# speechcatcher-asr/speechcatcher

Measured on AMD Instinct MI355X. Metric: concurrent real-time streams (audio-seconds/s), de_xl dims, 640 ms (10240-sample) chunk steps, beam 10 CTC+attention, higher is better.
Workload: dtype f32

## Files before the change

include/scasr.h:

```cpp
#ifndef SCASR_H
#define SCASR_H

#include <stddef.h>
#include <stdint.h>

#ifdef __cplusplus
extern "C" {
#endif

#define SC_OK 0
#define SC_ERR_ARG (-1)
#define SC_ERR_LAUNCH (-2)
#define SC_ERR_CAPACITY (-3)
#define SC_ERR_INPUT (-4)

#define SC_GEMM_RELU 1
#define SC_GEMM_RESIDUAL 2
#define SC_GEMM_LN_AT_CROWS 8
#define SC_GEMM_NAIVE 4
#define SC_GEMM_SPLIT16 16

#define SC_F_ANY_EOS 1
#define SC_F_BEST_EOS 2
#define SC_F_ALL_EOS 4
// ... 321 lines not shown
int sc_align_hyps(sc_streams *streams, const int *stream_ids, int n, int nbest, int max_len, int32_t *start,
                  int32_t *end, float *logp_mean, double *path_score, int *status, int *n_hyps);
int sc_align_tokens(sc_streams *streams, int stream, const int32_t *ids, int L, int32_t *start, int32_t *end,
                    float *logp_mean, double *path_score, int *status);
int sc_reset(sc_streams *streams, int stream);
int sc_stream_info(const sc_streams *streams, int stream, sc_stream_info_t *out);
#define SC_KV_POOL_DEFAULT_MAX_GIB 24
int sc_streams_kv_rows(const sc_streams *streams);
int sc_streams_stats(const sc_streams *streams, long *enc_calls, long *dec_steps, long *dec_blocks);
int sc_streams_capture_stats(const sc_streams *streams, long *n_captures, double *seconds);
int sc_streams_set_graphs(sc_streams *streams, int on);
int sc_marker(int id, void *stream);
int sc_streams_host_times(sc_streams *streams, double *launch_s, double *wait_s);
int sc_streams_bucket_times(sc_streams *streams, double *seconds, long *iterations);
long sc_streams_take_xattn_rows(sc_streams *streams);
int sc_streams_take_xattn_rows_by_kernel(sc_streams *streams, long *rows);
int sc_streams_take_attn_counters(sc_streams *streams, long *out );
void *sc_streams_hip_stream(sc_streams *streams);
float *sc_streams_pcm(sc_streams *streams, long *capacity);
int sc_streams_write_pcm(sc_streams *streams, int stream, long offset, const float *host, long n);
long sc_streams_read_pcm_buffer(sc_streams *streams, int stream, float *host, long max_n);
int sc_streams_read_enc(sc_streams *streams, int stream, float *host, int max_frames);
int sc_streams_read_ctc(sc_streams *streams, int stream, float *host, int max_rows);

#ifdef __cplusplus
}
#endif
#endif
```

speechcatcher_amd/_abi.py:

```python
import ctypes as C
import os
import subprocess
from pathlib import Path

HERE = Path(__file__).resolve().parent
LIB_PATH = HERE / "libscasr.so"
CSRC = HERE / "csrc"

c_float_p = C.POINTER(C.c_float)
c_int_p = C.POINTER(C.c_int32)
c_double_p = C.POINTER(C.c_double)
vp = C.c_void_p


class EncLayer(C.Structure):
    _fields_ = [(n, vp) for n in ("ln1_g", "ln1_b", "wqkv", "bqkv", "wo", "bo",
                                  "ln2_g", "ln2_b", "w1", "b1", "w2", "b2", "w1_p", "w2_p",
                                  "wqkv_p", "wo_p", "w1_h", "w2_h", "wqkv_h", "wo_h", "w1_s", "w2_s",
                                  "wqkv_s", "wo_s")]


class DecLayer(C.Structure):
    _fields_ = [(n, vp) for n in ("ln1_g", "ln1_b", "wqkv", "bqkv", "wo", "bo",
                                  "ln2_g", "ln2_b", "wq", "bq", "wo2", "bo2",
# ... 154 lines not shown
    "sc_stream_last_error": (C.c_char_p, [vp, C.c_int]),
    "sc_reset": (C.c_int, [vp, C.c_int]),
    "sc_stream_info": (C.c_int, [vp, C.c_int, C.POINTER(StreamInfo)]),
    "sc_streams_stats": (C.c_int, [vp, C.POINTER(C.c_long), C.POINTER(C.c_long), C.POINTER(C.c_long)]),
    "sc_streams_capture_stats": (C.c_int, [vp, C.POINTER(C.c_long), c_double_p]),
    "sc_streams_set_graphs": (C.c_int, [vp, C.c_int]),
    "sc_marker": (C.c_int, [C.c_int, vp]),
    "sc_streams_host_times": (C.c_int, [vp, c_double_p, c_double_p]),
    "sc_streams_bucket_times": (C.c_int, [vp, c_double_p, C.POINTER(C.c_long)]),
    "sc_streams_take_xattn_rows": (C.c_long, [vp]),
    "sc_streams_take_xattn_rows_by_kernel": (C.c_int, [vp, vp]),
    "sc_streams_take_attn_counters": (C.c_int, [vp, vp]),
    "sc_streams_hip_stream": (vp, [vp]),
    "sc_streams_pcm": (vp, [vp, C.POINTER(C.c_long)]),
    "sc_streams_write_pcm": (C.c_int, [vp, C.c_int, C.c_long, vp, C.c_long]),
    "sc_streams_read_pcm_buffer": (C.c_long, [vp, C.c_int, vp, C.c_long]),
    "sc_streams_read_enc": (C.c_int, [vp, C.c_int, vp, C.c_int]),
    "sc_ctc_align_ws_bytes": (C.c_size_t, [C.c_int]),
    "sc_ctc_align": (C.c_int, [vp, C.c_int, C.c_int, C.c_int, vp]),
    "sc_align_hyps": (C.c_int, [vp, c_int_p, C.c_int, C.c_int, C.c_int, c_int_p, c_int_p, c_float_p, c_double_p,
                                c_int_p, c_int_p]),
    "sc_align_tokens": (C.c_int, [vp, C.c_int, c_int_p, C.c_int, c_int_p, c_int_p, c_float_p, c_double_p, c_int_p]),
    "sc_streams_read_ctc": (C.c_int, [vp, C.c_int, vp, C.c_int]),
}

EXPORTED_SYMBOLS = tuple(_SIGS.keys())

ABI_VERSION = 7

_lib = None


class ScasrError(RuntimeError):
    pass


def build(verbose: bool = False) -> Path:
    cmd = ["make", "-C", str(CSRC), "-j4"]
    res = subprocess.run(cmd, capture_output=True, text=True)
    if verbose or res.returncode != 0:
        print(res.stdout)
        print(res.stderr)
    if res.returncode != 0:
        raise ScasrError("building libscasr.so failed")
    return LIB_PATH

# ... 32 lines not shown
```

speechcatcher_amd/csrc/common.h:

```cpp
#pragma once
#include <hip/hip_runtime.h>
#include <stdint.h>
#include <stdio.h>
#include <math.h>

#include "../../include/scasr.h"

#define SC_LOGZERO (-10000000000.0f)

void sc_set_error(const char *fmt, ...);

const char *sc_hook(const char *name);

__attribute__((visibility("hidden"))) int allow_large_lds(const void *fn, size_t need, size_t max_bytes, const char *what);

#define SC_CHECK_ARG(cond, msg)      \
  do {                               \
    if (!(cond)) {                   \
      sc_set_error("%s: %s", __func__, msg); \
      return SC_ERR_ARG;             \
    }                                \
  } while (0)

#define SC_CHECK_LAUNCH()                                              \
// ... 16 lines not shown
  __attribute__((visibility("hidden"))) ~ProfScope() {
    if (on) { (void)hipEventDestroy(a); (void)hipEventDestroy(b); }
  }
};
ProfScope sc_prof_begin(hipStream_t st);
void sc_prof_end(ProfScope &p, int kind, double flops, double bytes);

int sc_decode_step_form(const sc_search *sb);
int sc_gemm_colblocks(const float *A, const int32_t *a_rows, int lda, const float *W, const float *bias, float *C,
                      const int32_t *c_rows, int ldc, int M, int N, int K, int ncb, long cb_stride, int flags, void *stream);

int sc_dec_layer_hpw(const sc_search &sb);
int sc_dec_layer_stream_form(const sc_search &sb);
int sc_dec_layer_split_ffn(const sc_search &sb);

int sc_launch_reduce_ln_proj(const float *part, int npart, int part_M, const float *b2, const float *Xin, float *Xout,
                             const int32_t *rows, int M, int D, const float *ln_g, const float *ln_b, float ln_eps,
                             float *XN, const float *Wq, const float *bq, float *Q, int N, hipStream_t st,
                             int by_row = 0, int half_mode = 0);

struct ScHandoff { const int32_t *blkinfo; int R; float *state; int layer; };
int sc_ffn_ln_handoff(const float *XN, int M, int D, int F, const void *W1, const float *b1, const void *W2, const float *b2,
                      float *X, int w_form, const ScHandoff &ho, void *stream);

template <int CTRL>
__device__ __forceinline__ float dpp_mov(float v) {
  return __int_as_float(__builtin_amdgcn_update_dpp(0, __float_as_int(v), CTRL, 0xF, 0xF, true));
}
#define SC_DPP_XOR1 0xB1
#define SC_DPP_XOR2 0x4E
#define SC_DPP_HALF_MIRROR 0x141
#define SC_DPP_ROR4 0x124
#define SC_DPP_ROR8 0x128
#define SC_DPP_ROW_MIRROR 0x140

template <int LPR>
__device__ __forceinline__ float group_sum(float v) {
  v += dpp_mov<SC_DPP_XOR1>(v);
  v += dpp_mov<SC_DPP_XOR2>(v);
  if (LPR >= 8) v += dpp_mov<SC_DPP_HALF_MIRROR>(v);
  if (LPR == 16) v += dpp_mov<SC_DPP_ROW_MIRROR>(v);
  return v;
}

__device__ __forceinline__ float sc_lane(float v, int lane) {
  return __int_as_float(__builtin_amdgcn_readlane(__float_as_int(v), lane));
// ... 108 lines not shown
```

speechcatcher_amd/csrc/encoder.hip:

```cpp
#include "common.h"
#include <stdarg.h>
#include <string.h>

static thread_local char g_err[512] = "";
void sc_set_error(const char *fmt, ...) {
  va_list ap;
  va_start(ap, fmt);
  vsnprintf(g_err, sizeof(g_err), fmt, ap);
  va_end(ap);
}
extern "C" const char *sc_last_error(void) { return g_err; }
extern "C" int sc_version(void) { return SC_ABI_VERSION; }

template <int ID>
__global__ void sc_marker_kernel() {}
extern "C" int sc_marker(int id, void *stream) {
  hipStream_t st = (hipStream_t)stream;
  switch (id) {
    case 0: sc_marker_kernel<0><<<1, 64, 0, st>>>(); break;
    case 1: sc_marker_kernel<1><<<1, 64, 0, st>>>(); break;
    case 2: sc_marker_kernel<2><<<1, 64, 0, st>>>(); break;
    case 3: sc_marker_kernel<3><<<1, 64, 0, st>>>(); break;
    default: sc_set_error("sc_marker: id must be 0..3"); return SC_ERR_ARG;
  }
// ... 563 lines not shown
  const bool mfma = dk == 32 && R <= 48 && !(masked && R < 2) && !sp;
  if (mfma) {
    enc_attention_mfma_kernel<<<nblk * H, 256, 0, st>>>(qkv, att, nblk, R, H, d, masked);
  } else if (dk == 32 && split) {
    enc_attention_split_kernel<32><<<nblk * H, 256, 4 * 64 * (32 + 2) * sizeof(float), st>>>(qkv, att, nblk, R, H, d,
                                                                                            masked);
  } else if (dk == 16 && split) {
    enc_attention_split_kernel<16><<<nblk * H, 256, 4 * 64 * (16 + 2) * sizeof(float), st>>>(qkv, att, nblk, R, H, d,
                                                                                            masked);
  } else if (dk == 32) {
    enc_attention_kernel<32><<<grid, 256, 4 * 2 * 64 * 32 * sizeof(float), st>>>(qkv, att, nblk, R, H, d, masked);
  } else if (dk == 16) {
    enc_attention_kernel<16><<<grid, 256, 4 * 2 * 64 * 16 * sizeof(float), st>>>(qkv, att, nblk, R, H, d, masked);
  } else if (dk == 64) {
    enc_attention_kernel<64><<<grid, 256, 4 * 2 * 64 * 64 * sizeof(float), st>>>(qkv, att, nblk, R, H, d, masked);
  } else {
    sc_set_error("sc_enc_attention: unsupported head dim %d", dk);
    return SC_ERR_ARG;
  }
  SC_CHECK_LAUNCH();
  return SC_OK;
}

extern "C" int sc_encoder_layers(const sc_enc_layer *L, int n_layers, float *x, int nblk, int R,
                                 int masked, const int32_t *jobs, int ns, float *past_ctx,
                                 float *xn, float *qkv, float *att, float *ffh, int d, int H, int F,
                                 float eps, void *stream) {
  SC_CHECK_ARG(L && x && xn && qkv && att && ffh, "null pointer");
  const int M = nblk * R;
  if (M <= 0) return SC_OK;
  const bool ffn_fused = sc_ffn_ln_supported(d, F) && sc_workspace_bytes(stream) >= (size_t)(F / 128) * 80 * d * sizeof(float);
  const char *re = sc_hook("SC_ENC_ROWTILE");
  const bool rowtile_ok = sc_rowtile_proj_supported(d, d) && !(re && atoi(re) == 0);
  int rc;
  const bool fused_handoff = masked && ns > 0 && ffn_fused && R > 1 &&
                             sc_workspace_bytes(stream) >= (size_t)(F / 128) * M * d * sizeof(float) &&
                             (size_t)M * F >= (size_t)nblk * 4;
  int32_t *blkinfo = reinterpret_cast<int32_t *>(ffh);
  if (fused_handoff) {
    ctx_blkinfo_kernel<<<1, 256, 0, (hipStream_t)stream>>>(jobs, ns, nblk, blkinfo);
    SC_CHECK_LAUNCH();
  }
  for (int li = 0; li < n_layers; ++li) {
    const sc_enc_layer &w = L[li];
    const bool rowtile = rowtile_ok && w.wqkv_p && w.wo_p;
    const bool proj_h = rowtile && w.wqkv_h && w.wo_h;
    const bool proj_s = rowtile && w.wqkv_s && w.wo_s;
    if (proj_s) {
      SC_TRY(sc_rowtile_proj_s(x, d, M, d, w.ln1_g, w.ln1_b, eps, w.wqkv_s, w.bqkv, 3 * d, nullptr, qkv, 3 * d,
                               nullptr, nullptr, nullptr, stream));
    } else if (proj_h) {
      SC_TRY(sc_rowtile_proj_h(x, d, M, d, w.ln1_g, w.ln1_b, eps, w.wqkv_h, w.bqkv, 3 * d, nullptr, qkv, 3 * d,
                               nullptr, nullptr, nullptr, stream));
    } else if (rowtile) {
      SC_TRY(sc_rowtile_proj(x, d, M, d, w.ln1_g, w.ln1_b, eps, w.wqkv_p, w.bqkv, 3 * d, nullptr, qkv, 3 * d,
                             nullptr, nullptr, nullptr, stream));
    } else {
      SC_TRY(sc_layernorm(x, nullptr, d, xn, nullptr, d, M, d, w.ln1_g, w.ln1_b, eps, stream));
      SC_TRY(sc_gemm(xn, nullptr, d, w.wqkv, w.bqkv, qkv, nullptr, 3 * d, M, 3 * d, d, 0, 0, stream));
    }
    SC_TRY(sc_enc_attention(qkv, att, nblk, R, H, d, masked, stream));
    if (proj_s) {
      SC_TRY(sc_rowtile_proj_s(att, d, M, d, nullptr, nullptr, eps, w.wo_s, w.bo, d, x, x, d, w.ln2_g, w.ln2_b, xn,
                               stream));
    } else if (proj_h) {
      SC_TRY(sc_rowtile_proj_h(att, d, M, d, nullptr, nullptr, eps, w.wo_h, w.bo, d, x, x, d, w.ln2_g, w.ln2_b, xn,
                               stream));
    } else if (rowtile) {
      SC_TRY(sc_rowtile_proj(att, d, M, d, nullptr, nullptr, eps, w.wo_p, w.bo, d, x, x, d, w.ln2_g, w.ln2_b, xn,
                             stream));
    } else {
      SC_TRY(sc_gemm(att, nullptr, d, w.wo, w.bo, x, nullptr, d, M, d, d, SC_GEMM_RESIDUAL, 0, stream));
      SC_TRY(sc_layernorm(x, nullptr, d, xn, nullptr, d, M, d, w.ln2_g, w.ln2_b, eps, stream));
    }
    if (fused_handoff) {
      const int wf = (w.w1_s && w.w2_s) ? 2 : (w.w1_h && w.w2_h) ? 1 : 0;
      const ScHandoff ho{blkinfo, R, past_ctx, li};
      SC_TRY(sc_ffn_ln_handoff(xn, M, d, F, wf == 2 ? w.w1_s : wf == 1 ? w.w1_h : (const void *)w.w1_p, w.b1,
                               wf == 2 ? w.w2_s : wf == 1 ? w.w2_h : (const void *)w.w2_p, w.b2, x, wf, ho, stream));
      continue;
    }
    if (ffn_fused) {
      if (w.w1_s && w.w2_s)
        SC_TRY(sc_ffn_ln_s(xn, nullptr, M, d, F, w.w1_s, w.b1, w.w2_s, w.b2, x, nullptr, nullptr, eps, nullptr, stream));
      else if (w.w1_h && w.w2_h)
        SC_TRY(sc_ffn_ln_h(xn, nullptr, M, d, F, w.w1_h, w.b1, w.w2_h, w.b2, x, nullptr, nullptr, eps, nullptr, stream));
      else
        SC_TRY(sc_ffn_ln(xn, nullptr, M, d, F, w.w1_p, w.b1, w.w2_p, w.b2, x, nullptr, nullptr, eps, nullptr, stream));
    } else {
      SC_TRY(sc_gemm(xn, nullptr, d, w.w1, w.b1, ffh, nullptr, F, M, F, d, SC_GEMM_RELU, 0, stream));
      SC_TRY(sc_gemm(ffh, nullptr, F, w.w2, w.b2, x, nullptr, d, M, d, F, SC_GEMM_RESIDUAL, 0, stream));
    }
    if (masked && ns > 0) SC_TRY(sc_ctx_handoff(x, R, jobs, ns, past_ctx, li, d, stream));
  }
  return SC_OK;
}
```

speechcatcher_amd/csrc/streams.hip:

```cpp
#include <algorithm>
#include <array>
#include <chrono>
#include <cmath>
#include <cstdarg>
#include <cstring>
#include <deque>
#include <map>
#include <memory>
#include <new>
#include <string>
#include <vector>

#include "common.h"

namespace {

#define HIP_TRY(call)                                                              \
  do {                                                                             \
    hipError_t e__ = (call);                                                       \
    if (e__ != hipSuccess) {                                                       \
      sc_set_error("%s: %s failed: %s", __func__, #call, hipGetErrorString(e__));  \
      return SC_ERR_LAUNCH;                                                        \
    }                                                                              \
  } while (0)
// ... 119 lines not shown
  size_t stage_floats = 0;
  std::vector<int32_t> fe_jobs;
  int n_fe = 0, max_keep = 0;
  EncPlan P;
  std::vector<int32_t> ctc_rows, kv_src, kv_dst;
  bool same_rows = true;
  std::vector<int> streams;
  bool empty() const { return !n_fe && !P.n_conv; }
};

constexpr int N_ARENA = 8;
constexpr int N_STAGE = 4;
constexpr int N_RING = 4;

struct sc_streams {
  sc_engine *eng = nullptr;
  sc_config cfg{};
  int S = 0, W = 0, K = 0, TCAP = 0, LCAP = 0, FCAP = 0, UCAP = 0, max_feat_new = 0, max_t1 = 0, max_t2 = 0,
      max_blocks = 0, max_chunk = 0, max_length = 500;
  long PCAP = 0;
  bool use_bbd = false, strict = true;
  hipStream_t stream = nullptr;
  hipStream_t stream_enc = nullptr, es = nullptr;
  hipEvent_t ev_iter[2] = {nullptr, nullptr};
  int32_t *ring_dev = nullptr;
  int32_t *rm_host[2] = {nullptr, nullptr};
  int rm_idx = 0;
  bool rm_dirty = false;
  int scan_split_min = 1024, scan_split_streams = 0;
  bool scan_long = false;
  int step_split_min() const { return (scan_long && (scan_split_streams <= 0 || n_rows_step <= scan_split_streams * W)) ? scan_split_min : 0; }
  int graph_key() const { return n_rows_step * 2 + (step_split_min() > 0 ? 1 : 0); }
  int enc_start_thr = 0;
  int enc_batch_min = 0;
  int gemm_flags = 0;
  void *ws = nullptr, *ws_enc = nullptr;
  std::vector<void *> owned, owned_host;
  float *pcm = nullptr, *featbuf = nullptr, *subbuf = nullptr, *prev_addin = nullptr, *past_ctx = nullptr, *enc = nullptr,
        *c1 = nullptr, *c2 = nullptr, *xblk = nullptr, *ws_xn = nullptr, *ws_qkv = nullptr, *ws_att = nullptr,
        *ws_ffh = nullptr;
  int32_t *jobs_ctx = nullptr, *ctrlmap = nullptr;
  float *kv_stage = nullptr;
  int kv_stage_rows = 0;
  sc_search sb{};
  int32_t *ctrlmap_host = nullptr, *flags_host = nullptr;
  int32_t *arena_host = nullptr, *arena_dev = nullptr;
  size_t slot_cap = 0, arena_off = 0;
  int cur_slot = 0;
  hipEvent_t ev_group[N_ARENA] = {nullptr};
  long slot_gen[N_ARENA] = {0};
  int32_t *bs_host = nullptr, *bs_dev = nullptr;
  size_t bs_cap = 0;
  int bs_i = 0;
  float *stage_host = nullptr, *stage_dev = nullptr;
  size_t stage_cap = 0;
  hipEvent_t ev_stage[N_STAGE] = {nullptr};
  bool stage_busy[N_STAGE] = {false};
  int stage_next = 0;
  long long *cjobs_host = nullptr, *cjobs_dev = nullptr;
// ... 28 lines not shown
  std::vector<int> rowmap_key;
  int row_bucket = 1, n_rows_step = 0;
  bool decode_prepared = false;
  std::map<int, hipGraphExec_t> dec_graphs;
  std::map<std::vector<long>, hipGraphExec_t> enc_graphs;
  long dec_steps = 0, dec_blocks = 0, enc_calls = 0, xattn_rows[3] = {0, 0, 0};
  long sattn_pos[3] = {0, 0, 0};
  unsigned long long *stat_rows = nullptr;
  double t_launch = 0, t_wait = 0;
  double t_bucket[17] = {0};
  long n_bucket[17] = {0};
  bool use_graphs = true;
  long n_enc_captures = 0;
  double t_enc_capture = 0;

  ~sc_streams() {
    for (auto &g : dec_graphs) (void)hipGraphExecDestroy(g.second);
    for (auto &g : enc_graphs) (void)hipGraphExecDestroy(g.second);
    if (stream) (void)sc_set_stream_workspace(stream, nullptr, 0);
    if (stream_enc) {
      (void)sc_set_stream_workspace(stream_enc, nullptr, 0);
      (void)hipStreamDestroy(stream_enc);
    }
    for (int i = 0; i < 2; ++i)
      if (ev_iter[i]) (void)hipEventDestroy(ev_iter[i]);
    for (int i = 0; i < N_ARENA; ++i)
      if (ev_group[i]) (void)hipEventDestroy(ev_group[i]);
    for (int i = 0; i < N_STAGE; ++i)
      if (ev_stage[i]) (void)hipEventDestroy(ev_stage[i]);
    if (ev_snap) (void)hipEventDestroy(ev_snap);
    for (EncGroup *g : groups) delete g;
    for (void *p : owned) (void)hipFree(p);
    for (void *p : owned_host) (void)hipHostFree(p);
    if (stream_rb) (void)hipStreamDestroy(stream_rb);
    if (stream) (void)hipStreamDestroy(stream);
    if (al_dev) (void)hipFree(al_dev);
  }

  template <typename T>
  int alloc(T **p, size_t n) {
    RC_TRY(dalloc(p, n));
    owned.push_back(*p);
    return SC_OK;
  }
  template <typename T>
  int halloc(T **p, size_t n) {
// ... 267 lines not shown
    for (int i = 0; i < nb; ++i) {
      const int cur_hop = i * c.hop_size + (first ? offset : 0);
      const int clen = (i == nb - 1 && fin) ? std::min(c.block_size - offset, y_len - cur_hop) : c.hop_size;
      for (int j = 0; j < clen; ++j)
        if (cur_hop + j >= 0 && cur_hop + j < y_len) src[cur_hop + j] = (b0 + i) * R + 1 + offset + j;
    }
    if (st.T_enc + y_len > b->TCAP) throw StreamFault{s, SC_ERR_CAPACITY, "encoder-frame capacity exceeded (max_frames)"};
    for (int i = 0; i < y_len; ++i) {
      P.emit_src.push_back(src[i]);
      P.emit_dst.push_back(s * b->TCAP + st.T_enc + i);
    }
    st.T_enc += y_len;
    st.n_blocks += nb;
  }
  for (int s : streams)
    if (finals.at(s)) {
      St &st = b->st[s];
      st.enc_started = false;
      st.nfeat = st.nsub = st.n_blocks = 0;
      st.has_sub = st.has_addin = st.has_ctx = false;
    }
}

int enc_layers_launch(sc_streams *b, int nblk, int R, bool masked, const int32_t *jobs, int ns) {
  const sc_config &c = b->cfg;
  sc_engine *e = b->eng;
  auto launch = [&]() {
    return sc_encoder_layers(e->enc.data(), (int)e->enc.size(), b->xblk, nblk, R, masked ? 1 : 0, jobs, ns, b->past_ctx,
                             b->ws_xn, b->ws_qkv, b->ws_att, b->ws_ffh, c.d_model, c.enc_heads, c.ffn_dim, c.ln_eps,
                             b->es);
  };
  if (!b->use_graphs) return launch();
  std::vector<long> key{nblk, R, (long)masked, (long)(intptr_t)jobs, ns};
  auto it = b->enc_graphs.find(key);
  if (it == b->enc_graphs.end()) {
    if (b->enc_graphs.size() >= 192) return launch();
    const auto tc0 = std::chrono::steady_clock::now();
    RC_TRY(sc_graph_capture_begin(b->es));
    const int rc = launch();
    void *g = nullptr;
    const int rc2 = sc_graph_capture_end(b->es, &g);
    b->n_enc_captures++;
    b->t_enc_capture += std::chrono::duration<double>(std::chrono::steady_clock::now() - tc0).count();
    if (rc != SC_OK) return rc;
    if (rc2 != SC_OK) return rc2;
    it = b->enc_graphs.emplace(key, (hipGraphExec_t)g).first;
  }
  return sc_graph_launch(it->second, b->es);
}

int encode_short(sc_streams *b, const EncPlan::Short &sh) {
  const sc_config &c = b->cfg;
  sc_engine *e = b->eng;
  const int U = sh.U;
  const int32_t *jd, *src, *dst;
  RC_TRY(b->itensor({sh.ubase, U, sh.pe_pos, 0, 1, 0}, &jd));
  RC_TRY(sc_block_pack(b->subbuf, jd, 1, U, e->f("pe"), c.d_model, b->xblk, b->es));
  RC_TRY(sc_encoder_layers(e->enc.data(), (int)e->enc.size(), b->xblk, 1, U, 0, nullptr, 0, b->past_ctx, b->ws_xn,
                           b->ws_qkv, b->ws_att, b->ws_ffh, c.d_model, c.enc_heads, c.ffn_dim, c.ln_eps, b->es));
  std::vector<int32_t> a(U), d(U);
  for (int i = 0; i < U; ++i) { a[i] = i; d[i] = sh.s * b->TCAP + sh.dst_T + i; }
  RC_TRY(b->itensor(a, &src));
  RC_TRY(b->itensor(d, &dst));
  RC_TRY(sc_layernorm(b->xblk, src, c.d_model, b->enc, dst, c.d_model, U, c.d_model, e->f("enc_norm_g"), e->f("enc_norm_b"),
                      c.ln_eps, b->es));
  return SC_OK;
}

int encode_launch(sc_streams *b, EncPlan &P) {
  const sc_config &c = b->cfg;
  sc_engine *e = b->eng;
// ... 11 lines not shown
  if (!P.feat_src.empty()) {
    const int32_t *a, *z;
    RC_TRY(b->itensor(P.feat_src, &a));
    RC_TRY(b->itensor(P.feat_dst, &z));
    RC_TRY(sc_copy_rows(b->featbuf, a, b->featbuf, z, (int)P.feat_src.size(), c.n_mels, b->es));
  }
  const int nbk = (int)P.blk_jobs.size() / 6, ns = (int)P.sjobs.size() / 5;
  if (nbk > 0) {
    if (nbk > b->max_blocks) {
      sc_set_error("sc_push: too many encoder blocks in one call");
      return SC_ERR_ARG;
    }
    const int32_t *bj, *ja;
    RC_TRY(b->itensor(P.blk_jobs, &bj));
    RC_TRY(sc_block_pack(b->subbuf, bj, nbk, R, e->f("pe"), d, b->xblk, b->es));
    std::vector<int32_t> j_add(ns * 4), j_ctx(ns * 4);
    for (int i = 0; i < ns; ++i) {
      const int32_t *sj = &P.sjobs[i * 5];
      j_add[i * 4 + 0] = sj[0]; j_add[i * 4 + 1] = sj[1]; j_add[i * 4 + 2] = sj[2]; j_add[i * 4 + 3] = sj[3];
      j_ctx[i * 4 + 0] = sj[0]; j_ctx[i * 4 + 1] = sj[1]; j_ctx[i * 4 + 2] = sj[2] * c.enc_layers; j_ctx[i * 4 + 3] = sj[4];
    }
    RC_TRY(b->itensor(j_add, &ja));
    RC_TRY(sc_ctx_handoff(b->xblk, R, ja, ns, b->prev_addin, 0, d, b->es));
    const int32_t *jc;
    RC_TRY(b->itensor(j_ctx, &jc));
    HIP_TRY(hipMemcpyAsync(b->jobs_ctx, jc, j_ctx.size() * sizeof(int32_t), hipMemcpyDeviceToDevice, b->es));
    RC_TRY(enc_layers_launch(b, nbk, R, true, b->jobs_ctx, ns));
  }
  if (!P.emit_src.empty()) {
    const int32_t *a, *z;
    RC_TRY(b->itensor(P.emit_src, &a));
    RC_TRY(b->itensor(P.emit_dst, &z));
    RC_TRY(sc_layernorm(b->xblk, a, d, b->enc, z, d, (int)P.emit_src.size(), d, e->f("enc_norm_g"), e->f("enc_norm_b"),
                        c.ln_eps, b->es));
  }
  for (auto &sh : P.shorts) RC_TRY(encode_short(b, sh));
  if (!P.sub_src.empty()) {
    const int32_t *a, *z;
    RC_TRY(b->itensor(P.sub_src, &a));
    RC_TRY(b->itensor(P.sub_dst, &z));
    RC_TRY(sc_copy_rows(b->subbuf, a, b->subbuf, z, (int)P.sub_src.size(), d, b->es));
  }
  return SC_OK;
}

void set_rowmap(sc_streams *b, const std::vector<int> &active) {
  const int S = b->S, W = b->W;
  const int na = (int)active.size();
  const int nb = std::min(S, (na + b->row_bucket - 1) / b->row_bucket * b->row_bucket);
  if (active != b->rowmap_key) {
// ... 903 lines not shown
  if (hipStreamCreateWithPriority(&b->stream, hipStreamNonBlocking, -1) != hipSuccess) {
    sc_set_error("sc_streams_create: hipStreamCreate failed");
    delete b;
    return SC_ERR_LAUNCH;
  }
  if (hipStreamCreateWithPriority(&b->stream_rb, hipStreamNonBlocking, -1) != hipSuccess) {
    sc_set_error("sc_streams_create: hipStreamCreate failed");
    delete b;
    return SC_ERR_LAUNCH;
  }
  A(b->pcm, (size_t)S * b->PCAP);
  A(b->featbuf, (size_t)2 * S * b->FCAP * c.n_mels);
  A(b->subbuf, (size_t)2 * S * b->UCAP * d);
  A(b->prev_addin, (size_t)S * d);
  A(b->past_ctx, (size_t)S * c.enc_layers * d);
  A(b->enc, (size_t)S * b->TCAP * d);
  A(b->c1, (size_t)S * b->max_t1 * c.conv_freq1 * d);
  A(b->c2, (size_t)S * b->max_t2 * c.conv_freq2 * d);
  A(b->xblk, m_enc * d);
  A(b->ws_xn, m_enc * d);
  A(b->ws_qkv, m_enc * 3 * d);
  A(b->ws_att, m_enc * d);
  A(b->ws_ffh, m_enc * F);
  A(b->jobs_ctx, (size_t)S * 4);
  A(b->ctrlmap, (size_t)S * 8 + n);
  b->slot_cap = (((size_t)S * ((size_t)b->max_t2 * (c.conv_freq2 + 12) + 512) + 8192) + 63) & ~size_t(63);
  A(b->arena_dev, b->slot_cap * N_ARENA);
  b->bs_cap = (size_t)S * 8 + (size_t)S * c.block_size;
  A(b->bs_dev, b->bs_cap * N_RING);
  b->stage_cap = (size_t)S * std::max<size_t>((size_t)b->max_chunk + 16 * c.hop_length, (size_t)b->max_feat_new * c.n_mels);
  A(b->stage_dev, b->stage_cap * N_STAGE);
  b->pack_cap = n * (2 * (size_t)b->LCAP + 8);
  A(b->pack_dev, b->pack_cap);
  A(b->pjobs_dev, n * 4);
  A(b->cjobs_dev, (size_t)N_STAGE * S * 3);
  sc_search &sb = b->sb;
  sb.S = S; sb.W = W; sb.K = K; sb.V = V; sb.d = d; sb.H = c.dec_heads; sb.F = F; sb.n_layers = c.dec_layers;
  sb.TCAP = b->TCAP; sb.LCAP = b->LCAP; sb.blank = c.blank_id; sb.eos = c.eos_id; sb.sos = c.sos_id;
  sb.w_dec = 1.0f - o->ctc_weight; sb.w_ctc = o->ctc_weight; sb.ln_eps = c.ln_eps;
  float *ctcx = nullptr, *ckv = nullptr;
  A(ctcx, (size_t)S * b->TCAP * V);
  sb.kv_half = o->kv_half != 0;
  const size_t kvdiv = sb.kv_half ? 2 : 1;
  A(ckv, (size_t)S * c.dec_layers * b->TCAP * 2 * d / kvdiv + 4);
  sb.ctcx = ctcx; sb.ckv = ckv;
  if (sb.kv_half) {
    b->kv_stage_rows = std::max(256, S * 24);
// ... 67 lines not shown
  if (sb.kv_half && e->f("out_w_qh", false) && !e->dec.empty() && e->dec[0].wqkv_pph && e->dec[0].wq_pph && e->dec[0].wo_pph &&
      e->dec[0].wo2_pph && sb.ph1) {
    sb.out_w_qh = e->f("out_w_qh", false);
    sb.act_half = 1 | 2;
    if (const char *ah = sc_hook("SC_ACT_HALF")) sb.act_half = atoi(ah) & 7;
  }
  sb.layers = e->dec.data();
  (void)sc_set_stream_workspace(b->stream, b->ws, (size_t)128 << 20);
  b->es = b->stream;
  {
    b->enc_start_thr = S < 16 ? S : std::max(1, (int)((long)S * 7 / 100));
  }
  {
    const hipError_t er = hipStreamCreateWithPriority(&b->stream_enc, hipStreamNonBlocking, 0);
    if (er == hipSuccess && hipMalloc(&b->ws_enc, (size_t)128 << 20) == hipSuccess) {
      b->owned.push_back(b->ws_enc);
      (void)sc_set_stream_workspace(b->stream_enc, b->ws_enc, (size_t)128 << 20);
    } else {
      (void)hipGetLastError();
      if (b->stream_enc) (void)hipStreamDestroy(b->stream_enc);
      b->stream_enc = nullptr;
    }
  }
  const size_t cm = ((size_t)S * 8 + n) * sizeof(int32_t);
  bool ok = b->halloc(&b->ctrlmap_host, (size_t)S * 8 + n) == SC_OK && b->halloc(&b->flags_host, (size_t)S * 2) == SC_OK &&
            b->halloc(&b->rm_host[0], n) == SC_OK && b->halloc(&b->rm_host[1], n) == SC_OK &&
            b->halloc(&b->arena_host, b->slot_cap * N_ARENA) == SC_OK && b->halloc(&b->bs_host, b->bs_cap * N_RING) == SC_OK &&
            b->halloc(&b->stage_host, b->stage_cap * N_STAGE) == SC_OK && b->halloc(&b->pack_host, b->pack_cap) == SC_OK &&
            b->halloc(&b->pjobs_host, n * 4) == SC_OK && b->halloc(&b->cjobs_host, (size_t)N_STAGE * S * 3) == SC_OK;
  for (int i = 0; i < 2 && ok; ++i) ok = hipEventCreateWithFlags(&b->ev_iter[i], hipEventDisableTiming) == hipSuccess;
  for (int i = 0; i < N_ARENA && ok; ++i) ok = hipEventCreateWithFlags(&b->ev_group[i], hipEventDisableTiming) == hipSuccess;
  for (int i = 0; i < N_STAGE && ok; ++i) ok = hipEventCreateWithFlags(&b->ev_stage[i], hipEventDisableTiming) == hipSuccess;
  if (!ok) {
    sc_set_error("sc_streams_create: pinned host allocation failed");
    delete b;
    return SC_ERR_LAUNCH;
  }
  memset(b->flags_host, 0, (size_t)S * 8);
  {
    void *dv = nullptr;
    if (hipHostGetDevicePointer(&dv, b->flags_host, 0) != hipSuccess || !dv) {
      sc_set_error("sc_streams_create: pinned flags are not device-accessible");
      delete b;
      return SC_ERR_LAUNCH;
    }
    b->ring_dev = (int32_t *)dv;
// ... 11 lines not shown
  b->gemm_flags = (!b->eng->enc.empty() && b->eng->enc[0].wqkv_s) ? SC_GEMM_SPLIT16 : 0;
  b->row_bucket = std::max(1, S / 32);
  b->n_rows_step = S * W;
  b->st.assign(S, St());
  b->run.assign(S, Run());
  b->bq.assign(S, std::deque<Blk>());
  b->job.assign(S, Job());
  b->ahead.assign(S, std::deque<Job>());
  b->job_seq.assign(S, 0);
  b->snap.assign(S, Snap());
  b->done_at.assign(S, 0);
  b->fault_msg.assign(S, std::string());
  b->enc_gen.assign(S, 0);
  for (int s = 0; s < S; ++s) init_hyp(b, s);
  *out = b;
  return SC_OK;
  SC_API_END
}

extern "C" void sc_streams_destroy(sc_streams *b) {
  if (b) {
    (void)hipStreamSynchronize(b->stream);
    if (b->stream_enc) (void)hipStreamSynchronize(b->stream_enc);
    delete b;
  }
}

extern "C" int sc_reset(sc_streams *b, int stream) {
  SC_CHECK_ARG(b && stream >= 0 && stream < b->S, "stream out of range");
  SC_CHECK_ARG(!b->job[stream].open, "the stream has a chunk outstanding (sc_poll reports it first)");
  reset_stream(b, stream);
  return SC_OK;
}

extern "C" void *sc_streams_hip_stream(sc_streams *b) { return b ? (void *)b->stream : nullptr; }

extern "C" float *sc_streams_pcm(sc_streams *b, long *capacity) {
  if (!b) return nullptr;
  if (capacity) *capacity = b->PCAP;
  return b->pcm;
}

namespace {

int report_chunk(sc_streams *b, int s) {
  Job &j = b->job[s];
// ... 444 lines not shown
  return retire_groups(b);
}
extern "C" long sc_streams_read_pcm_buffer(sc_streams *b, int stream, float *host, long max_n) {
  if (!b || stream < 0 || stream >= b->S) return SC_ERR_ARG;
  if (settle_encoder(b) != SC_OK) return SC_ERR_LAUNCH;
  const St &st = b->st[stream];
  const long n = std::min<long>(st.pcm_end - st.pcm_start, max_n);
  if (host && n > 0 &&
      hipMemcpy(host, b->pcm + (long)stream * b->PCAP + st.pcm_start, (size_t)n * sizeof(float), hipMemcpyDeviceToHost) != hipSuccess)
    return SC_ERR_LAUNCH;
  return n;
}
extern "C" int sc_streams_read_enc(sc_streams *b, int stream, float *host, int max_frames) {
  if (!b || stream < 0 || stream >= b->S) return SC_ERR_ARG;
  if (settle_encoder(b) != SC_OK) return SC_ERR_LAUNCH;
  const int T = std::min(b->st[stream].T_enc, max_frames);
  if (host && T > 0 &&
      hipMemcpy(host, b->enc + (size_t)stream * b->TCAP * b->cfg.d_model, (size_t)T * b->cfg.d_model * sizeof(float),
                hipMemcpyDeviceToHost) != hipSuccess)
    return SC_ERR_LAUNCH;
  return T;
}

extern "C" int sc_streams_read_ctc(sc_streams *b, int stream, float *host, int max_rows) {
  SC_CHECK_ARG(b && stream >= 0 && stream < b->S && max_rows >= 0, "bad arguments");
  SC_API_BEGIN
  HIP_TRY(hipSetDevice(b->eng->device));
  int T = 0;
  bool snap = false;
  RC_TRY(hyp_frames(b, stream, &T, &snap));
  T = std::min(T, max_rows);
  const size_t V = (size_t)b->cfg.vocab_size;
  if (host && T > 0) {
    HIP_TRY(hipMemcpyAsync(host, b->sb.ctcx + (size_t)stream * b->TCAP * V, (size_t)T * V * sizeof(float),
                           hipMemcpyDeviceToHost, b->stream_rb));
    HIP_TRY(hipStreamSynchronize(b->stream_rb));
  }
  return T;
  SC_API_END
}

extern "C" int sc_stream_info(const sc_streams *b, int stream, sc_stream_info_t *out) {
  SC_CHECK_ARG(b && out && stream >= 0 && stream < b->S, "bad arguments");
  const St &st = b->st[stream];
  out->enc_frames = st.T_enc;
  out->processed_block = st.processed_block;
// ... 82 lines not shown
```

speechcatcher_amd/native.py:

```python
import ctypes as C
from typing import Optional, Sequence, Tuple

import numpy as np
import torch

from . import _abi
from .config import SearchConfig
from .engine import EngineError
from .weights import PackedWeights

_ERR_CAPACITY, _ERR_INPUT = -3, -4


class NativeEngine:

    def __init__(self, weights: Optional[PackedWeights] = None, packed_path: Optional[str] = None, device="cuda:0"):
        self.lib = _abi.load()
        self.device = torch.device(device)
        h = C.c_void_p()
        if packed_path is not None:
            _abi.check(self.lib.sc_engine_load(str(packed_path).encode(), self.device.index or 0, C.byref(h)),
                       "sc_engine_load")
            self.weights = None
        else:
# ... 263 lines not shown
                                          ps.ctypes.data_as(_abi.c_double_p), st.ctypes.data_as(ip),
                                          nh.ctypes.data_as(ip)), "sc_align_hyps")
        return {"start": start, "end": end, "logp_mean": lp, "path_score": ps, "status": st, "n_hyps": nh}

    def align_tokens(self, s: int, ids: Sequence[int]):
        y = np.ascontiguousarray(ids, dtype=np.int32)
        L = y.shape[0]
        start, end = np.zeros(max(L, 1), np.int32), np.zeros(max(L, 1), np.int32)
        lp = np.zeros(max(L, 1), np.float32)
        ps, st = C.c_double(0.0), C.c_int32(0)
        ip = _abi.c_int_p
        _abi.check(self.lib.sc_align_tokens(self.handle, int(s), y.ctypes.data_as(ip), L, start.ctypes.data_as(ip),
                                            end.ctypes.data_as(ip), lp.ctypes.data_as(_abi.c_float_p), C.byref(ps),
                                            C.byref(st)), "sc_align_tokens")
        return {"start": start[:L], "end": end[:L], "logp_mean": lp[:L], "path_score": ps.value, "status": st.value}

    def read_ctc(self, s: int) -> np.ndarray:
        a = np.zeros((self.TCAP, self.cfg.vocab_size), np.float32)
        T = self.lib.sc_streams_read_ctc(self.handle, int(s), a.ctypes.data, self.TCAP)
        if T < 0:
            _abi.check(T, "sc_streams_read_ctc")
        return a[:T].copy()

    def hypotheses_batch(self, streams: Sequence[int], nbest: Optional[int] = None):
        a = self.hypotheses_arrays(streams, nbest)
        out = {}
        for i, s in enumerate(streams):
            hy = []
            for j in range(int(a["n_hyps"][i])):
                L = int(a["lens"][i, j])
                hy.append({"yseq": a["ids"][i, j, :L].tolist(), "score": float(a["score"][i, j]),
                           "score_dec": float(a["score_dec"][i, j]), "score_ctc": float(a["score_ctc"][i, j]),
                           "xpos": a["xpos"][i, j, :L].tolist()})
            out[int(s)] = hy
        return out

    def hypotheses(self, s: int):
        return self.hypotheses_batch([int(s)])[int(s)]

    def write_pcm(self, s: int, offset: int, samples: np.ndarray):
        a = np.ascontiguousarray(samples, dtype=np.float32)
        _abi.check(self.lib.sc_streams_write_pcm(self.handle, int(s), int(offset), a.ctypes.data, a.shape[0]),
                   "sc_streams_write_pcm")

    def waveform_buffer(self, s: int) -> np.ndarray:
        n = self.st[s].pcm_buffered
# ... 49 lines not shown
```

Measured before the change: 4071.

## Split batched encoder layers across two concurrent HIP streams with staggered head

```diff
diff --git a/include/scasr.h b/include/scasr.h
--- a/include/scasr.h
+++ b/include/scasr.h
@@ -367,6 +367,7 @@
 long sc_streams_read_pcm_buffer(sc_streams *streams, int stream, float *host, long max_n);
 int sc_streams_read_enc(sc_streams *streams, int stream, float *host, int max_frames);
 int sc_streams_read_ctc(sc_streams *streams, int stream, float *host, int max_rows);
+int sc_streams_read_state(sc_streams *streams, int stream, int what, void *host, int max_rows);
 
 #ifdef __cplusplus
 }
diff --git a/speechcatcher_amd/_abi.py b/speechcatcher_amd/_abi.py
--- a/speechcatcher_amd/_abi.py
+++ b/speechcatcher_amd/_abi.py
@@ -200,6 +200,7 @@
                                 c_int_p, c_int_p]),
     "sc_align_tokens": (C.c_int, [vp, C.c_int, c_int_p, C.c_int, c_int_p, c_int_p, c_float_p, c_double_p, c_int_p]),
     "sc_streams_read_ctc": (C.c_int, [vp, C.c_int, vp, C.c_int]),
+    "sc_streams_read_state": (C.c_int, [vp, C.c_int, C.c_int, vp, C.c_int]),
 }
 
 EXPORTED_SYMBOLS = tuple(_SIGS.keys())
diff --git a/speechcatcher_amd/csrc/common.h b/speechcatcher_amd/csrc/common.h
--- a/speechcatcher_amd/csrc/common.h
+++ b/speechcatcher_amd/csrc/common.h
@@ -62,6 +62,11 @@
 struct ScHandoff { const int32_t *blkinfo; int R; float *state; int layer; };
 int sc_ffn_ln_handoff(const float *XN, int M, int D, int F, const void *W1, const float *b1, const void *W2, const float *b2,
                       float *X, int w_form, const ScHandoff &ho, void *stream);
+
+enum { SC_ENC_ALL = 0, SC_ENC_HEAD = 1, SC_ENC_REST = 2 };
+int sc_encoder_layers_part(const sc_enc_layer *L, int n_layers, float *x, int nblk, int R, int masked, const int32_t *jobs,
+                           int ns, float *past_ctx, float *xn, float *qkv, float *att, float *ffh, int d, int H, int F,
+                           float eps, int part, void *stream);
 
 template <int CTRL>
 __device__ __forceinline__ float dpp_mov(float v) {
diff --git a/speechcatcher_amd/csrc/encoder.hip b/speechcatcher_amd/csrc/encoder.hip
--- a/speechcatcher_amd/csrc/encoder.hip
+++ b/speechcatcher_amd/csrc/encoder.hip
@@ -609,10 +609,9 @@
   return SC_OK;
 }
 
-extern "C" int sc_encoder_layers(const sc_enc_layer *L, int n_layers, float *x, int nblk, int R,
-                                 int masked, const int32_t *jobs, int ns, float *past_ctx,
-                                 float *xn, float *qkv, float *att, float *ffh, int d, int H, int F,
-                                 float eps, void *stream) {
+int sc_encoder_layers_part(const sc_enc_layer *L, int n_layers, float *x, int nblk, int R, int masked, const int32_t *jobs,
+                           int ns, float *past_ctx, float *xn, float *qkv, float *att, float *ffh, int d, int H, int F,
+                           float eps, int part, void *stream) {
   SC_CHECK_ARG(L && x && xn && qkv && att && ffh, "null pointer");
   const int M = nblk * R;
   if (M <= 0) return SC_OK;
@@ -624,7 +623,7 @@
                              sc_workspace_bytes(stream) >= (size_t)(F / 128) * M * d * sizeof(float) &&
                              (size_t)M * F >= (size_t)nblk * 4;
   int32_t *blkinfo = reinterpret_cast<int32_t *>(ffh);
-  if (fused_handoff) {
+  if (fused_handoff && part != SC_ENC_REST) {
     ctx_blkinfo_kernel<<<1, 256, 0, (hipStream_t)stream>>>(jobs, ns, nblk, blkinfo);
     SC_CHECK_LAUNCH();
   }
@@ -633,33 +632,36 @@
     const bool rowtile = rowtile_ok && w.wqkv_p && w.wo_p;
     const bool proj_h = rowtile && w.wqkv_h && w.wo_h;
     const bool proj_s = rowtile && w.wqkv_s && w.wo_s;
-    if (proj_s) {
-      SC_TRY(sc_rowtile_proj_s(x, d, M, d, w.ln1_g, w.ln1_b, eps, w.wqkv_s, w.bqkv, 3 * d, nullptr, qkv, 3 * d,
+    if (part != SC_ENC_REST || li > 0) {
+      if (proj_s) {
+        SC_TRY(sc_rowtile_proj_s(x, d, M, d, w.ln1_g, w.ln1_b, eps, w.wqkv_s, w.bqkv, 3 * d, nullptr, qkv, 3 * d,
+                                 nullptr, nullptr, nullptr, stream));
+      } else if (proj_h) {
+        SC_TRY(sc_rowtile_proj_h(x, d, M, d, w.ln1_g, w.ln1_b, eps, w.wqkv_h, w.bqkv, 3 * d, nullptr, qkv, 3 * d,
+                                 nullptr, nullptr, nullptr, stream));
+      } else if (rowtile) {
+        SC_TRY(sc_rowtile_proj(x, d, M, d, w.ln1_g, w.ln1_b, eps, w.wqkv_p, w.bqkv, 3 * d, nullptr, qkv, 3 * d,
                                nullptr, nullptr, nullptr, stream));
-    } else if (proj_h) {
-      SC_TRY(sc_rowtile_proj_h(x, d, M, d, w.ln1_g, w.ln1_b, eps, w.wqkv_h, w.bqkv, 3 * d, nullptr, qkv, 3 * d,
-                               nullptr, nullptr, nullptr, stream));
-    } else if (rowtile) {
-      SC_TRY(sc_rowtile_proj(x, d, M, d, w.ln1_g, w.ln1_b, eps, w.wqkv_p, w.bqkv, 3 * d, nullptr, qkv, 3 * d,
-                             nullptr, nullptr, nullptr, stream));
-    } else {
-      SC_TRY(sc_layernorm(x, nullptr, d, xn, nullptr, d, M, d, w.ln1_g, w.ln1_b, eps, stream));
-      SC_TRY(sc_gemm(xn, nullptr, d, w.wqkv, w.bqkv, qkv, nullptr, 3 * d, M, 3 * d, d, 0, 0, stream));
-    }
-    SC_TRY(sc_enc_attention(qkv, att, nblk, R, H, d, masked, stream));
-    if (proj_s) {
-      SC_TRY(sc_rowtile_proj_s(att, d, M, d, nullptr, nullptr, eps, w.wo_s, w.bo, d, x, x, d, w.ln2_g, w.ln2_b, xn,
+      } else {
+        SC_TRY(sc_layernorm(x, nullptr, d, xn, nullptr, d, M, d, w.ln1_g, w.ln1_b, eps, stream));
+        SC_TRY(sc_gemm(xn, nullptr, d, w.wqkv, w.bqkv, qkv, nullptr, 3 * d, M, 3 * d, d, 0, 0, stream));
+      }
+      SC_TRY(sc_enc_attention(qkv, att, nblk, R, H, d, masked, stream));
+      if (proj_s) {
+        SC_TRY(sc_rowtile_proj_s(att, d, M, d, nullptr, nullptr, eps, w.wo_s, w.bo, d, x, x, d, w.ln2_g, w.ln2_b, xn,
+                                 stream));
+      } else if (proj_h) {
+        SC_TRY(sc_rowtile_proj_h(att, d, M, d, nullptr, nullptr, eps, w.wo_h, w.bo, d, x, x, d, w.ln2_g, w.ln2_b, xn,
+                                 stream));
+      } else if (rowtile) {
+        SC_TRY(sc_rowtile_proj(att, d, M, d, nullptr, nullptr, eps, w.wo_p, w.bo, d, x, x, d, w.ln2_g, w.ln2_b, xn,
                                stream));
-    } else if (proj_h) {
-      SC_TRY(sc_rowtile_proj_h(att, d, M, d, nullptr, nullptr, eps, w.wo_h, w.bo, d, x, x, d, w.ln2_g, w.ln2_b, xn,
-                               stream));
-    } else if (rowtile) {
-      SC_TRY(sc_rowtile_proj(att, d, M, d, nullptr, nullptr, eps, w.wo_p, w.bo, d, x, x, d, w.ln2_g, w.ln2_b, xn,
-                             stream));
-    } else {
-      SC_TRY(sc_gemm(att, nullptr, d, w.wo, w.bo, x, nullptr, d, M, d, d, SC_GEMM_RESIDUAL, 0, stream));
-      SC_TRY(sc_layernorm(x, nullptr, d, xn, nullptr, d, M, d, w.ln2_g, w.ln2_b, eps, stream));
-    }
+      } else {
+        SC_TRY(sc_gemm(att, nullptr, d, w.wo, w.bo, x, nullptr, d, M, d, d, SC_GEMM_RESIDUAL, 0, stream));
+        SC_TRY(sc_layernorm(x, nullptr, d, xn, nullptr, d, M, d, w.ln2_g, w.ln2_b, eps, stream));
+      }
+    }
+    if (part == SC_ENC_HEAD) break;
     if (fused_handoff) {
       const int wf = (w.w1_s && w.w2_s) ? 2 : (w.w1_h && w.w2_h) ? 1 : 0;
       const ScHandoff ho{blkinfo, R, past_ctx, li};
@@ -682,3 +684,11 @@
   }
   return SC_OK;
 }
+
+extern "C" int sc_encoder_layers(const sc_enc_layer *L, int n_layers, float *x, int nblk, int R,
+                                 int masked, const int32_t *jobs, int ns, float *past_ctx,
+                                 float *xn, float *qkv, float *att, float *ffh, int d, int H, int F,
+                                 float eps, void *stream) {
+  return sc_encoder_layers_part(L, n_layers, x, nblk, R, masked, jobs, ns, past_ctx, xn, qkv, att, ffh, d, H, F, eps, SC_ENC_ALL,
+                                stream);
+}
diff --git a/speechcatcher_amd/csrc/streams.hip b/speechcatcher_amd/csrc/streams.hip
--- a/speechcatcher_amd/csrc/streams.hip
+++ b/speechcatcher_amd/csrc/streams.hip
@@ -165,6 +165,11 @@
   bool use_bbd = false, strict = true;
   hipStream_t stream = nullptr;
   hipStream_t stream_enc = nullptr, es = nullptr;
+  hipStream_t stream_enc2 = nullptr;
+  hipEvent_t ev_fork = nullptr, ev_join = nullptr;
+  int enc_chains = 1;
+  bool enc_stagger = true;
+  int enc_chain_min_blocks = 16;
   hipEvent_t ev_iter[2] = {nullptr, nullptr};
   int32_t *ring_dev = nullptr;
   int32_t *rm_host[2] = {nullptr, nullptr};
@@ -177,7 +182,7 @@
   int enc_start_thr = 0;
   int enc_batch_min = 0;
   int gemm_flags = 0;
-  void *ws = nullptr, *ws_enc = nullptr;
+  void *ws = nullptr, *ws_enc = nullptr, *ws_enc2 = nullptr;
   std::vector<void *> owned, owned_host;
   float *pcm = nullptr, *featbuf = nullptr, *subbuf = nullptr, *prev_addin = nullptr, *past_ctx = nullptr, *enc = nullptr,
         *c1 = nullptr, *c2 = nullptr, *xblk = nullptr, *ws_xn = nullptr, *ws_qkv = nullptr, *ws_att = nullptr,
@@ -252,6 +257,12 @@
       (void)sc_set_stream_workspace(stream_enc, nullptr, 0);
       (void)hipStreamDestroy(stream_enc);
     }
+    if (stream_enc2) {
+      (void)sc_set_stream_workspace(stream_enc2, nullptr, 0);
+      (void)hipStreamDestroy(stream_enc2);
+    }
+    if (ev_fork) (void)hipEventDestroy(ev_fork);
+    if (ev_join) (void)hipEventDestroy(ev_join);
     for (int i = 0; i < 2; ++i)
       if (ev_iter[i]) (void)hipEventDestroy(ev_iter[i]);
     for (int i = 0; i < N_ARENA; ++i)
@@ -565,31 +576,57 @@
     }
 }
 
-int enc_layers_launch(sc_streams *b, int nblk, int R, bool masked, const int32_t *jobs, int ns) {
+int enc_layers_launch(sc_streams *b, int blk0, int nblk, int R, bool masked, const int32_t *jobs, int ns, int part,
+                      hipStream_t st) {
   const sc_config &c = b->cfg;
   sc_engine *e = b->eng;
+  const size_t r0 = (size_t)blk0 * R;
   auto launch = [&]() {
-    return sc_encoder_layers(e->enc.data(), (int)e->enc.size(), b->xblk, nblk, R, masked ? 1 : 0, jobs, ns, b->past_ctx,
-                             b->ws_xn, b->ws_qkv, b->ws_att, b->ws_ffh, c.d_model, c.enc_heads, c.ffn_dim, c.ln_eps,
-                             b->es);
+    return sc_encoder_layers_part(e->enc.data(), (int)e->enc.size(), b->xblk + r0 * c.d_model, nblk, R, masked ? 1 : 0, jobs, ns,
+                                  b->past_ctx, b->ws_xn + r0 * c.d_model, b->ws_qkv + r0 * 3 * c.d_model,
+                                  b->ws_att + r0 * c.d_model, b->ws_ffh + r0 * c.ffn_dim, c.d_model, c.enc_heads, c.ffn_dim,
+                                  c.ln_eps, part, st);
   };
   if (!b->use_graphs) return launch();
-  std::vector<long> key{nblk, R, (long)masked, (long)(intptr_t)jobs, ns};
+  std::vector<long> key{nblk, R, (long)masked, (long)(intptr_t)jobs, ns, blk0, part, (long)(intptr_t)st};
   auto it = b->enc_graphs.find(key);
   if (it == b->enc_graphs.end()) {
-    if (b->enc_graphs.size() >= 192) return launch();
+    if (b->enc_graphs.size() >= 576) return launch();
     const auto tc0 = std::chrono::steady_clock::now();
-    RC_TRY(sc_graph_capture_begin(b->es));
+    RC_TRY(sc_graph_capture_begin(st));
     const int rc = launch();
     void *g = nullptr;
-    const int rc2 = sc_graph_capture_end(b->es, &g);
+    const int rc2 = sc_graph_capture_end(st, &g);
     b->n_enc_captures++;
     b->t_enc_capture += std::chrono::duration<double>(std::chrono::steady_clock::now() - tc0).count();
     if (rc != SC_OK) return rc;
     if (rc2 != SC_OK) return rc2;
     it = b->enc_graphs.emplace(key, (hipGraphExec_t)g).first;
   }
-  return sc_graph_launch(it->second, b->es);
+  return sc_graph_launch(it->second, st);
+}
+
+int enc_chains_launch(sc_streams *b, int nblk, int R, std::vector<int32_t> &j_ctx, int ns) {
+  int cut = 0;
+  if (b->stream_enc2 && b->es == b->stream_enc && b->enc_chains >= 2 && nblk >= b->enc_chain_min_blocks)
+    for (int i = 1; i < ns; ++i)
+      if (cut == 0 || std::abs(2 * j_ctx[i * 4] - nblk) < std::abs(2 * j_ctx[cut * 4] - nblk)) cut = i;
+  const int nblkA = cut ? j_ctx[cut * 4] : nblk, nsA = cut ? cut : ns;
+  for (int i = cut; cut && i < ns; ++i) j_ctx[i * 4] -= nblkA;
+  const int32_t *jc;
+  RC_TRY(b->itensor(j_ctx, &jc));
+  HIP_TRY(hipMemcpyAsync(b->jobs_ctx, jc, (size_t)nsA * 4 * sizeof(int32_t), hipMemcpyDeviceToDevice, b->es));
+  if (!cut) return enc_layers_launch(b, 0, nblk, R, true, b->jobs_ctx, ns, SC_ENC_ALL, b->es);
+  int32_t *jobsB = b->jobs_ctx + (size_t)b->S * 4;
+  HIP_TRY(hipMemcpyAsync(jobsB, jc + nsA * 4, (size_t)(ns - nsA) * 4 * sizeof(int32_t), hipMemcpyDeviceToDevice, b->es));
+  if (b->enc_stagger) RC_TRY(enc_layers_launch(b, 0, nblkA, R, true, b->jobs_ctx, nsA, SC_ENC_HEAD, b->es));
+  HIP_TRY(hipEventRecord(b->ev_fork, b->es));
+  HIP_TRY(hipStreamWaitEvent(b->stream_enc2, b->ev_fork, 0));
+  RC_TRY(enc_layers_launch(b, 0, nblkA, R, true, b->jobs_ctx, nsA, b->enc_stagger ? SC_ENC_REST : SC_ENC_ALL, b->es));
+  RC_TRY(enc_layers_launch(b, nblkA, nblk - nblkA, R, true, jobsB, ns - nsA, SC_ENC_ALL, b->stream_enc2));
+  HIP_TRY(hipEventRecord(b->ev_join, b->stream_enc2));
+  HIP_TRY(hipStreamWaitEvent(b->es, b->ev_join, 0));
+  return SC_OK;
 }
 
 int encode_short(sc_streams *b, const EncPlan::Short &sh) {
@@ -647,10 +684,7 @@
     }
     RC_TRY(b->itensor(j_add, &ja));
     RC_TRY(sc_ctx_handoff(b->xblk, R, ja, ns, b->prev_addin, 0, d, b->es));
-    const int32_t *jc;
-    RC_TRY(b->itensor(j_ctx, &jc));
-    HIP_TRY(hipMemcpyAsync(b->jobs_ctx, jc, j_ctx.size() * sizeof(int32_t), hipMemcpyDeviceToDevice, b->es));
-    RC_TRY(enc_layers_launch(b, nbk, R, true, b->jobs_ctx, ns));
+    RC_TRY(enc_chains_launch(b, nbk, R, j_ctx, ns));
   }
   if (!P.emit_src.empty()) {
     const int32_t *a, *z;
@@ -1600,7 +1634,7 @@
   A(b->ws_qkv, m_enc * 3 * d);
   A(b->ws_att, m_enc * d);
   A(b->ws_ffh, m_enc * F);
-  A(b->jobs_ctx, (size_t)S * 4);
+  A(b->jobs_ctx, (size_t)2 * S * 4);
   A(b->ctrlmap, (size_t)S * 8 + n);
   b->slot_cap = (((size_t)S * ((size_t)b->max_t2 * (c.conv_freq2 + 12) + 512) + 8192) + 63) & ~size_t(63);
   A(b->arena_dev, b->slot_cap * N_ARENA);
@@ -1714,6 +1748,27 @@
       b->stream_enc = nullptr;
     }
   }
+  {
+    int chains = b->enc_chains, stagger = 1, min_blocks = b->enc_chain_min_blocks;
+    if (const char *ec = sc_hook("SC_ENC_CHAINS")) (void)sscanf(ec, "%d,%d,%d", &chains, &stagger, &min_blocks);
+    b->enc_chains = chains;
+    b->enc_stagger = stagger != 0;
+    b->enc_chain_min_blocks = std::max(2, min_blocks);
+    if (b->stream_enc && chains >= 2) {
+      bool ok2 = chains != 3 && hipStreamCreateWithPriority(&b->stream_enc2, hipStreamNonBlocking, 0) == hipSuccess &&
+                 hipMalloc(&b->ws_enc2, (size_t)128 << 20) == hipSuccess;
+      if (ok2) b->owned.push_back(b->ws_enc2);
+      ok2 = ok2 && hipEventCreateWithFlags(&b->ev_fork, hipEventDisableTiming) == hipSuccess &&
+            hipEventCreateWithFlags(&b->ev_join, hipEventDisableTiming) == hipSuccess;
+      if (ok2) {
+        (void)sc_set_stream_workspace(b->stream_enc2, b->ws_enc2, (size_t)128 << 20);
+      } else {
+        (void)hipGetLastError();
+        if (b->stream_enc2) (void)hipStreamDestroy(b->stream_enc2);
+        b->stream_enc2 = nullptr;
+      }
+    }
+  }
   const size_t cm = ((size_t)S * 8 + n) * sizeof(int32_t);
   bool ok = b->halloc(&b->ctrlmap_host, (size_t)S * 8 + n) == SC_OK && b->halloc(&b->flags_host, (size_t)S * 2) == SC_OK &&
             b->halloc(&b->rm_host[0], n) == SC_OK && b->halloc(&b->rm_host[1], n) == SC_OK &&
@@ -1771,6 +1826,7 @@
   if (b) {
     (void)hipStreamSynchronize(b->stream);
     if (b->stream_enc) (void)hipStreamSynchronize(b->stream_enc);
+    if (b->stream_enc2) (void)hipStreamSynchronize(b->stream_enc2);
     delete b;
   }
 }
@@ -2261,6 +2317,29 @@
   return T;
 }
 
+extern "C" int sc_streams_read_state(sc_streams *b, int stream, int what, void *host, int max_rows) {
+  SC_CHECK_ARG(b && stream >= 0 && stream < b->S && max_rows >= 0 && (what == 0 || what == 1), "bad arguments");
+  SC_API_BEGIN
+  HIP_TRY(hipSetDevice(b->eng->device));
+  RC_TRY(settle_encoder(b));
+  const sc_config &c = b->cfg;
+  if (what == 0) {
+    const int n = std::min(c.enc_layers, max_rows);
+    if (host && n > 0)
+      HIP_TRY(hipMemcpy(host, b->past_ctx + (size_t)stream * c.enc_layers * c.d_model, (size_t)n * c.d_model * sizeof(float),
+                        hipMemcpyDeviceToHost));
+    return n;
+  }
+  const int T = std::min(b->st[stream].T_projkv, max_rows);
+  const size_t row = (size_t)2 * c.d_model * (b->sb.kv_half ? 2 : 4);
+  for (int li = 0; host && T > 0 && li < c.dec_layers; ++li)
+    HIP_TRY(hipMemcpy((char *)host + (size_t)li * T * row,
+                      (const char *)b->sb.ckv + ((size_t)stream * c.dec_layers + li) * b->TCAP * row, (size_t)T * row,
+                      hipMemcpyDeviceToHost));
+  return T;
+  SC_API_END
+}
+
 extern "C" int sc_streams_read_ctc(sc_streams *b, int stream, float *host, int max_rows) {
   SC_CHECK_ARG(b && stream >= 0 && stream < b->S && max_rows >= 0, "bad arguments");
   SC_API_BEGIN
diff --git a/speechcatcher_amd/native.py b/speechcatcher_amd/native.py
--- a/speechcatcher_amd/native.py
+++ b/speechcatcher_amd/native.py
@@ -309,6 +309,19 @@
             _abi.check(T, "sc_streams_read_ctc")
         return a[:T].copy()
 
+    def read_state(self, s: int):
+        ctx = np.zeros((self.cfg.enc_layers, self.cfg.d_model), np.float32)
+        n = self.lib.sc_streams_read_state(self.handle, int(s), 0, ctx.ctypes.data, self.cfg.enc_layers)
+        if n < 0:
+            _abi.check(n, "sc_streams_read_state")
+        T = self.lib.sc_streams_read_state(self.handle, int(s), 1, None, self.TCAP)
+        if T < 0:
+            _abi.check(T, "sc_streams_read_state")
+        kv = np.zeros((self.cfg.dec_layers, T, 2 * self.cfg.d_model), np.float16 if self.kv_dtype == "float16" else np.float32)
+        if T:
+            self.lib.sc_streams_read_state(self.handle, int(s), 1, kv.ctypes.data, T)
+        return ctx, kv
+
     def hypotheses_batch(self, streams: Sequence[int], nbest: Optional[int] = None):
         a = self.hypotheses_arrays(streams, nbest)
         out = {}
```

Result: no change. 4058 (-0.3%).
